# Liz490/multimodal_alzheimer

Hardware: AMD Instinct MI355X
Metric: volumes/sec fwd+bwd, 3D-ResNet-10 @128^3 bf16, 1/2/4/8 MI355X; % HBM roofline (higher is better)
Workload: dtype bf16; 1 GPU; BASELINE config 2: Anat_CNN ResNet-10 MRI-only, 1x128^3, batch 8/GPU, weighted CE, Adam, fwd+bwd+step; global_batch=8, parallelism=dp1, step_launch=hip graph replay

## Files before the change

### multimodal_alzheimer_amd/csrc/conv.hip

```cpp
#include <cstring>

#include "common.h"
#include "reduce.h"
#include "patchconv.h"
#include "pointwise.h"
#include "stem.h"

namespace {

constexpr int MAXTAPS = 344;
constexpr int TAPB = ((3 * MAXTAPS * 4 + 15) / 16) * 16;
constexpr int RB = 128;

struct Geom {
  int M, Nd, Cs, K, Kpad, cs_shift, taps, nb;
  int Ds, Hs, Ws, Dd, Hd, Wd;
  int KD, KH, KW;
  int sd, sh, sw, pd, ph, pw, dd, dh, dw;
  const void* res;
  int relu;
};

enum { FWD = 0, DGRAD = 1 };

// ... 1271 lines not shown
        return launch_igemm_bm<T, 128, MODE, 256, 4, 2, 2>(g, m_max, classes, src, w, bias,
                                                          dst, stats, st);
      if (cfg == 5)
        return launch_igemm_bm<T, 256, MODE, 256, 2, 4, 4, 64>(g, m_max, classes, src, w, bias,
                                                              dst, stats, st);
      if (cfg == 6)
        return launch_igemm_bm<T, 256, MODE, 256, 2, 4, 3, 64>(g, m_max, classes, src, w, bias,
                                                              dst, stats, st);
    }
  }
  const bool small = igemm_bm(m_max * classes, g) == 64;
  if constexpr (sizeof(T) == 2) {
    if (igemm_nst(g, MODE) == 3) {
      if (bn_of(g) == 64)
        return small ? launch_igemm_bm<T, 64, MODE, 64, 2, 2, 3>(g, m_max, classes, src, w, bias, dst, stats, st)
                     : launch_igemm_bm<T, 64, MODE, 128, 2, 2, 3>(g, m_max, classes, src, w, bias, dst, stats, st);
      return small ? launch_igemm_bm<T, 128, MODE, 64, 2, 2, 3>(g, m_max, classes, src, w, bias, dst, stats, st)
                   : launch_igemm_bm<T, 128, MODE, 128, 2, 2, 3>(g, m_max, classes, src, w, bias, dst, stats, st);
    }
  }
  if (bn_of(g) == 64)
    return small ? launch_igemm_bm<T, 64, MODE, 64>(g, m_max, classes, src, w, bias, dst, stats, st)
                 : launch_igemm_bm<T, 64, MODE, 128>(g, m_max, classes, src, w, bias, dst, stats, st);
  return small ? launch_igemm_bm<T, 128, MODE, 64>(g, m_max, classes, src, w, bias, dst, stats, st)
               : launch_igemm_bm<T, 128, MODE, 128>(g, m_max, classes, src, w, bias, dst, stats, st);
}

template <int MODE>
int run_igemm(const Geom& g, int dtype, int64_t m_max, int classes, const void* src,
              const void* w, const float* bias, void* dst, float* stats, hipStream_t st) {
  if (dtype == MMAD_BF16)
    return run_igemm_t<u16, MODE>(g, m_max, classes, src, w, bias, dst, stats, st);
  return run_igemm_t<float, MODE>(g, m_max, classes, src, w, bias, dst, stats, st);
}

int wgrad_xcd() {
  static const int v = [] { const char* e = getenv("MMAD_WGRAD_XCD"); return e ? atoi(e) : 1; }();
  return v;
}

template <typename T, int BMW, int WBK, int NST, int WBNT, int WGM, int WGN, bool XFIX>
int launch_wgrad_x(const Geom& g, const WSplit& sp, const void* x, const void* dy, float* ws,
                   hipStream_t st) {
  const size_t lds = TAPB + NST * WBK * (BMW + WBNT) * sizeof(T);
  static const bool ok = set_lds(wgrad_kernel<T, BMW, WBK, NST, WBNT, WGM, WGN, XFIX>, lds);
  if (!ok) return MMAD_EUNSUPPORTED;
  const uint32_t xb = (uint32_t)((int64_t)g.nb * g.Ds * g.Hs * g.Ws * g.Cs * sizeof(T));
  const uint32_t yb = (uint32_t)((int64_t)g.M * g.Nd * sizeof(T));
  dim3 grid((unsigned)cdiv(g.K, WBNT), (unsigned)cdiv(g.Nd, BMW), (unsigned)sp.splits);
  hipLaunchKernelGGL((wgrad_kernel<T, BMW, WBK, NST, WBNT, WGM, WGN, XFIX>), grid,
                     dim3(64 * WGM * WGN), lds, st, g, (const T*)x, (const T*)dy, ws,
                     sp.m_per_split, xb, yb, wgrad_xcd());
  return launch_status();
}

template <typename T, int BMW, int WBK, int NST, int WBNT = WBN, int WGM = 2, int WGN = 2>
int launch_wgrad_k(const Geom& g, const WSplit& sp, const void* x, const void* dy, float* ws,
                   hipStream_t st) {
  if ((int64_t)g.nb * g.Ds * g.Hs * g.Ws * g.Cs * (int64_t)sizeof(T) >= (int64_t(1) << 31) ||
      (int64_t)g.M * g.Nd * (int64_t)sizeof(T) >= (int64_t(1) << 31))
    return MMAD_EUNSUPPORTED;
  if (WBK % g.Wd == 0)
    return launch_wgrad_x<T, BMW, WBK, NST, WBNT, WGM, WGN, true>(g, sp, x, dy, ws, st);
  return launch_wgrad_x<T, BMW, WBK, NST, WBNT, WGM, WGN, false>(g, sp, x, dy, ws, st);
}

int wgrad_1x1_nst() {
  static const int v = [] { const char* e = getenv("MMAD_WGRAD_1X1_NST"); return e ? atoi(e) : 3; }();
  return v;
}

template <typename T, int BMW>
int launch_wgrad(const Geom& g, const WSplit& sp, const void* x, const void* dy, float* ws,
                 hipStream_t st) {
  if (g.taps == 1 && wgrad_1x1_nst() == 3) return launch_wgrad_k<T, BMW, 32, 3>(g, sp, x, dy, ws, st);
  return launch_wgrad_k<T, BMW, 32, 2>(g, sp, x, dy, ws, st);
}

unsigned grid_for(int64_t total, int block = 256) {
  return (unsigned)std::max<int64_t>(1, std::min<int64_t>(cdiv(total, block), 65536));
}

enum Leaf { STEM, LATTICE5, LATTICE_ZP, LATTICE, LATTICE8, PATCHZ, PATCH, S2, PW, IGEMM, NONE };
enum Epi { EPI_NONE, EPI_RES, EPI_BNSUM };
bool leaf_has(Leaf l, Epi e) {
  if (e == EPI_RES) return l != STEM && l != PW;
  if (e == EPI_BNSUM) return l == LATTICE_ZP || l == LATTICE8 || l == PATCH;
  return true;
}
struct Route { Leaf leaf; int64_t tiles; };

Route resolve(const mmad_conv_desc* d, const Geom& g, int dtype, Epi epi, bool launch = true) {
  const Route none{NONE, -1};
  auto pick = [&](Leaf l, int64_t tiles) { return leaf_has(l, epi) ? Route{l, tiles} : none; };
  const bool u = d != nullptr && unfolded(d);
  if (u && epi != EPI_NONE) return none;
  if (u && mmad_stem::fwd_ok(d, dtype) && stem_kernel_on())
    return pick(STEM, mmad_stem::fwd_stats_rows(d));
  if (launch && !geom_ok(g, dtype)) return none;
  if (!u && dtype == MMAD_BF16) {
    const mmad_patch::Geo q = patch_geo(g);
    if (g.sd == 1 && g.sh == 1 && g.sw == 1) {
      if (mmad_lattice5::ok(q)) return pick(LATTICE5, mmad_lattice5::tiles(q));
      const bool zp = mmad_lattice_zp::ok(q);
      const int64_t lt = zp ? mmad_lattice_zp::tiles(q) : mmad_lattice::tiles(q);
      if (mmad_lattice::ok(q, lt)) return pick(zp ? LATTICE_ZP : LATTICE, lt);
      if (mmad_lattice8::ok(q)) return pick(LATTICE8, mmad_lattice8::tiles(q));
      if (mmad_patch::ok(q))
        return mmad_patchz::ok(q) ? pick(PATCHZ, mmad_patchz::tiles(q))
                                  : pick(PATCH, mmad_patch::tiles(q));
    }
    if (mmad_s2::ok(q, g.sd, g.sh, g.sw)) return pick(S2, mmad_s2::tiles(q));
  }
  if (d != nullptr && leaf_has(PW, epi) && mmad_pw::fwd_ok(d, dtype))
    return pick(PW, mmad_pw::fwd_tiles(d));
  return pick(IGEMM, cdiv(g.M, fwd_tile_rows(g, dtype)));
}

int launch_route(const Route& r, const mmad_conv_desc* d, const Geom& g, int dtype,
                 const mmad_patch::Geo& q, const void* x, const void* wp, const float* bias,
                 void* y, float* stats, void* stream) {
  switch (r.leaf) {
    case STEM: return mmad_stem::fwd(d, x, wp, bias, y, stats, stream);
    case LATTICE5: return mmad_lattice5::fwd(q, x, wp, bias, y, stats, stream);
    case LATTICE_ZP: return mmad_lattice_zp::fwd(q, x, wp, bias, y, stats, stream);
    case LATTICE: return mmad_lattice::fwd(q, x, wp, bias, y, stats, stream);
    case LATTICE8: return mmad_lattice8::fwd(q, x, wp, bias, y, stats, stream);
    case PATCHZ: return mmad_patchz::fwd(q, x, wp, bias, y, stats, stream);
    case PATCH: return mmad_patch::fwd(q, x, wp, bias, y, stats, stream);
    case S2: return mmad_s2::fwd(q, g.sd, g.sh, g.sw, x, wp, bias, y, stats, stream);
    case PW: return mmad_pw::fwd(d, x, wp, bias, y, stats, stream);
    case IGEMM: return run_igemm<FWD>(g, dtype, g.M, 1, x, wp, bias, y, stats, as_stream(stream));
    case NONE: break;
  }
  return MMAD_EUNSUPPORTED;
}

Route dgrad_fwd_route(const mmad_conv_desc* d, int dtype, Epi epi, Geom* gf) {
  if (!desc_ok(d) || (dtype != MMAD_F32 && dtype != MMAD_BF16) || unfolded(d) ||
      mmad_pw::ok(d, dtype) || !dgrad_as_fwd(d))
    return Route{NONE, -1};
  *gf = dgrad_fwd_geom(d, dtype);
  return resolve(nullptr, *gf, dtype, epi);
}

}

extern "C" {

int mmad_set_kernel_variant(const char* name, int value) {
  if (name == nullptr) return -1;
  if (std::strcmp(name, "lattice_zp") == 0) return mmad_lattice_zp::set_mode(value);
  if (std::strcmp(name, "lattice") == 0) return mmad_lattice::set_mode(value);
  if (std::strcmp(name, "lattice8") == 0) return mmad_lattice8::set_mode(value);
  if (std::strcmp(name, "lattice8_xwalk") == 0) return mmad_lattice8::set_xwalk(value);
  if (std::strcmp(name, "lattice5") == 0) return mmad_lattice5::set_mode(value);
  if (std::strcmp(name, "pool_run") == 0) return mmad_pool::set_run_mode(value);
  if (std::strcmp(name, "patchz") == 0) return mmad_patchz::set_mode(value);
  if (std::strcmp(name, "pw_wg3_dedup") == 0) return mmad_pw::set_wg3_dedup(value);
  return -1;
}

int64_t mmad_conv_packed_elems(const mmad_conv_desc* d, int dtype, int for_dgrad) {
  if (!desc_ok(d)) return -1;
  const Geom g = for_dgrad ? dgrad_geom(d, dtype) : fwd_geom(d, dtype);
  return (int64_t)g.Nd * g.Kpad;
}

int mmad_conv_pack_weight_scaled(const mmad_conv_desc* d, int dtype, const float* w,
                                 const float* scale, void* wp, int for_dgrad, void* stream);

int mmad_conv_pack_weight(const mmad_conv_desc* d, int dtype, const float* w, void* wp,
                          int for_dgrad, void* stream) {
  return mmad_conv_pack_weight_scaled(d, dtype, w, nullptr, wp, for_dgrad, stream);
}

int mmad_conv_pack_weight_scaled(const mmad_conv_desc* d, int dtype, const float* w,
                                 const float* scale, void* wp, int for_dgrad, void* stream) {
  if (!desc_ok(d)) return MMAD_EBADSHAPE;
  if (dtype != MMAD_F32 && dtype != MMAD_BF16) return MMAD_EBADDTYPE;
  if (!w || !wp) return MMAD_ENULL;
  if (for_dgrad && unfolded(d)) return MMAD_EUNSUPPORTED;
  const Geom g = for_dgrad ? dgrad_geom(d, dtype) : fwd_geom(d, dtype);
  if (!geom_ok(g, dtype)) return MMAD_EUNSUPPORTED;
  const int mode = for_dgrad ? 1 : (unfolded(d) ? 2 : 0);
  const int flip = for_dgrad && dgrad_as_fwd(d);
  const int64_t total = (int64_t)g.Nd * g.Kpad;
  if (scale != nullptr && (mode != 0 || g.Kpad != g.K)) return MMAD_EUNSUPPORTED;
  if (mode != 2 && g.Kpad == g.K) {
    const int R = mode == 0 ? d->ci : d->co;
    const int Cc = mode == 0 ? g.taps : d->ci * g.taps;
    const int B = mode == 0 ? d->co : 1;
    const int64_t ob = mode == 0 ? g.Kpad : 0, oj1 = mode == 0 ? 0 : g.Kpad;
    const int jd = g.taps, oj2 = mode == 0 ? d->ci : d->co;
    dim3 grid((unsigned)cdiv(Cc, 64), (unsigned)cdiv(R, 64), (unsigned)B);
    if (dtype == MMAD_BF16)
      hipLaunchKernelGGL(pack_transpose_kernel<u16>, grid, dim3(256), 0, as_stream(stream), w,
                         (u16*)wp, R, Cc, ob, jd, oj1, oj2, flip, scale);
    else
      hipLaunchKernelGGL(pack_transpose_kernel<float>, grid, dim3(256), 0, as_stream(stream), w,
                         (float*)wp, R, Cc, ob, jd, oj1, oj2, flip, scale);
    return launch_status();
  }
  if (dtype == MMAD_BF16)
    hipLaunchKernelGGL(pack_weight_kernel<u16>, dim3(grid_for(total)), dim3(256), 0,
                       as_stream(stream), w, (u16*)wp, g.Nd, g.Kpad, g.K, g.Cs, g.cs_shift,
                       g.taps, mode, d->ci, d->kw, flip);
  else
    hipLaunchKernelGGL(pack_weight_kernel<float>, dim3(grid_for(total)), dim3(256), 0,
                       as_stream(stream), w, (float*)wp, g.Nd, g.Kpad, g.K, g.Cs, g.cs_shift,
                       g.taps, mode, d->ci, d->kw, flip);
  return launch_status();
}

int mmad_conv_pack_job(const mmad_conv_desc* d, int dtype, int for_dgrad, const float* w,
                       void* wp, int64_t tile0, mmad_pack_job* job) {
  if (!desc_ok(d)) return MMAD_EBADSHAPE;
  if (dtype != MMAD_F32 && dtype != MMAD_BF16) return MMAD_EBADDTYPE;
  if (!w || !wp || !job) return MMAD_ENULL;
  if (unfolded(d)) return MMAD_EUNSUPPORTED;
  const Geom g = for_dgrad ? dgrad_geom(d, dtype) : fwd_geom(d, dtype);
  if (!geom_ok(g, dtype) || g.Kpad != g.K) return MMAD_EUNSUPPORTED;
  const bool fw = !for_dgrad;
  mmad_pack_job j{};
  j.w = w;
  j.w_packed = wp;
  j.rows = fw ? d->co * d->ci : d->co;
  j.rdiv = fw ? d->ci : d->co;
  j.cols = fw ? g.taps : d->ci * g.taps;
  j.batch = 1;
  j.jdiv = g.taps;
  j.ostride_j2 = fw ? d->ci : d->co;
  j.ostride_b = fw ? g.Kpad : 0;
  j.ostride_j1 = fw ? 0 : g.Kpad;
  const bool narrow = j.cols <= 32;
  j.tiles_x = (int)cdiv(j.cols, narrow ? 32 : 64);
  j.tiles_y = (int)cdiv(j.rows, narrow ? 128 : 64);
  j.pad_ = for_dgrad && dgrad_as_fwd(d);
  j.tile0 = tile0;
  *job = j;
  return MMAD_OK;
}

int mmad_conv_pack_dual_job(const mmad_conv_desc* d, int dtype, const float* w, void* w_fwd,
                            void* w_dgrad, int64_t tile0, mmad_pack_dual* job) {
  if (!desc_ok(d)) return MMAD_EBADSHAPE;
  if (dtype != MMAD_BF16) return MMAD_EUNSUPPORTED;
  if (!w || !w_fwd || !w_dgrad || !job) return MMAD_ENULL;
  if (unfolded(d)) return MMAD_EUNSUPPORTED;
  const Geom gf = fwd_geom(d, dtype), gd = dgrad_geom(d, dtype);
  if (!geom_ok(gf, dtype) || !geom_ok(gd, dtype) || gf.Kpad != gf.K || gd.Kpad != gd.K)
    return MMAD_EUNSUPPORTED;
  if (d->ci % 16 || d->co % 16 || gf.taps > 27) return MMAD_EUNSUPPORTED;
  mmad_pack_dual j{};
  j.w = w;
  j.w_fwd = w_fwd;
  j.w_dgrad = w_dgrad;
  j.co = d->co;
  j.ci = d->ci;
  j.taps = gf.taps;
  j.flip = dgrad_as_fwd(d) ? 1 : 0;
  j.tile0 = tile0;
  *job = j;
  return MMAD_OK;
}

int64_t mmad_pack_dual_tiles(const mmad_pack_dual* job) {
  return job ? (int64_t)(job->co / 16) * (job->ci / 16) : -1;
}

int mmad_conv_pack_dual_batch(int dtype, int njobs, const mmad_pack_dual* jobs,
                              int64_t total_tiles, void* stream) {
  if (njobs <= 0 || total_tiles <= 0 || total_tiles > INT32_MAX) return MMAD_EBADSHAPE;
  if (!jobs) return MMAD_ENULL;
  if (dtype != MMAD_BF16) return MMAD_EBADDTYPE;
  hipLaunchKernelGGL(pack_dual_kernel, dim3((unsigned)total_tiles), dim3(256), 0,
                     as_stream(stream), jobs, njobs);
  return launch_status();
}

int64_t mmad_pack_job_tiles(const mmad_pack_job* job) {
  return job ? (int64_t)job->tiles_x * job->tiles_y * job->batch : -1;
}

int mmad_conv_pack_batch(int dtype, int njobs, const mmad_pack_job* jobs, int64_t total_tiles,
                         void* stream) {
  if (njobs <= 0 || total_tiles <= 0 || total_tiles > INT32_MAX) return MMAD_EBADSHAPE;
  if (!jobs) return MMAD_ENULL;
  if (dtype == MMAD_BF16)
    hipLaunchKernelGGL(pack_batch_kernel<u16>, dim3((unsigned)total_tiles), dim3(256), 0,
                       as_stream(stream), jobs, njobs);
  else if (dtype == MMAD_F32)
    hipLaunchKernelGGL(pack_batch_kernel<float>, dim3((unsigned)total_tiles), dim3(256), 0,
                       as_stream(stream), jobs, njobs);
  else
    return MMAD_EBADDTYPE;
  return launch_status();
}

int64_t mmad_conv_unfolded_elems(const mmad_conv_desc* d) {
  if (!desc_ok(d) || !unfolded(d)) return -1;
  return (int64_t)d->n * d->di * d->hi * d->wo * 8;
}

int mmad_conv_unfold_input(const mmad_conv_desc* d, int in_dtype, const void* x, int dtype,
                           void* xu, void* stream) {
// ... 379 lines not shown
```

### multimodal_alzheimer_amd/csrc/latticeconv.hip

```cpp
#include <algorithm>
#include <atomic>
#include <cstdlib>
#include <type_traits>

#include "common.h"
#include "patchconv.h"

namespace {

constexpr int S = 4;
constexpr int NS = 32;
constexpr int PL = S * S * NS;
constexpr int RBL = 64;
constexpr int KC = RBL / 2;
constexpr int PLANE = PL * RBL;
constexpr int BNL = 128;
constexpr int TPS = 3;
constexpr int BTAP = BNL * RBL;
constexpr int BSLOT = TPS * BTAP;
#ifndef LAT_NSTL
#define LAT_NSTL 3
#endif
constexpr int NSTL = LAT_NSTL;
constexpr int NPS = 2;
// ... 202 lines not shown
  };
  auto run = [&](auto wmc) {
    constexpr int WM = decltype(wmc)::value;
    for (int u = 0; u < ngrp; ++u) {
      const char* apl = smem + (u % NPS) * PLANE + a_lane;
      const int s0 = u * 3;
      const bool py = u >= 1 && u + 1 < ngrp;
      one_stage(s0, std::integral_constant<int, 0>{}, py);
      stage_body<TN, WM, -1>(acc, ring + (s0 % NSTL) * BSLOT + b_lane, apl);
      one_stage(s0 + 1, std::integral_constant<int, 1>{}, py);
      stage_body<TN, WM, 0>(acc, ring + ((s0 + 1) % NSTL) * BSLOT + b_lane, apl);
      one_stage(s0 + 2, std::integral_constant<int, 2>{}, py);
      stage_body<TN, WM, 1>(acc, ring + ((s0 + 2) % NSTL) * BSLOT + b_lane, apl);
    }
  };
  if (g.prio && wave >= 4) __builtin_amdgcn_s_setprio(1);
  switch (wm) {
    case 0: run(std::integral_constant<int, 0>{}); break;
    case 1: run(std::integral_constant<int, 1>{}); break;
    case 2: run(std::integral_constant<int, 2>{}); break;
    default: run(std::integral_constant<int, 3>{}); break;
  }
  __syncthreads();

  auto dst_vox = [&](int row) -> int64_t {
    const int pos = row / NS, s = row % NS;
    const int q = q0 + s;
    const int rz = q / (d * d), ry = (q / d) % d, rx = q % d;
    const int ty = pos / S, tx = pos % S;
    if constexpr (RAG) {
      const int z = rz + d * tz, y = ry + d * ty, x = rx + d * tx;
      if (z >= g.D || y >= g.H || x >= g.W) return -1;
      return (((int64_t)n * g.D + z) * g.H + y) * g.W + x;
    }
    return (((int64_t)n * E + rz + d * tz) * E + ry + d * ty) * E + rx + d * tx;
  };
  u16* ctile = reinterpret_cast<u16*>(smem);
  uint32_t vmask = 0xffffffffu;
  if constexpr (RAG) {
    vmask = 0;
#pragma unroll 1
    for (int b = 0; b < 32; ++b) {
      const int i = b >> 3, h = (b >> 2) & 1, e = b & 3;
      const int row = (i * S + ((i + wm) & 3)) * NS + h * 16 + lk * 4 + e;
      if (dst_vox(row) >= 0) vmask |= 1u << b;
    }
  }
  float cs[TN], cq[TN];
#pragma unroll
  for (int j = 0; j < TN; ++j) {
    cs[j] = 0.f;
    cq[j] = 0.f;
    const int col = wn * 16 * TN + j * 16 + lr;
    const float bv = bias != nullptr ? bias[n0 + col] : 0.f;
#pragma unroll
    for (int i = 0; i < 4; ++i) {
      const int pos = i * S + ((i + wm) & 3);
#pragma unroll
      for (int h = 0; h < 2; ++h)
#pragma unroll
        for (int e = 0; e < 4; ++e) {
          const int row = pos * NS + h * 16 + lk * 4 + e;
          const float v = acc[i * 2 + h][j][e] + bv;
          ctile[row * (CROW / 2) + col] = f2bf(v);
          if ((vmask >> (i * 8 + h * 4 + e)) & 1u) {
            cs[j] += v;
            cq[j] += v * v;
          }
        }
    }
  }
  __syncthreads();
  constexpr int CPR = BW / 8;
#pragma unroll
  for (int hh = 0; hh < PL * CPR / NTHR; ++hh) {
    const int qd = tid + NTHR * hh;
    const int row = qd / CPR, c8 = qd % CPR;
    const int64_t dv = dst_vox(row);
    if (RAG && dv < 0) continue;
    const int64_t o = dv * g.Nd + n0 + c8 * 8;
    u32x4 v = *reinterpret_cast<const u32x4*>(reinterpret_cast<const char*>(ctile) + row * CROW +
                                              c8 * 16);
    if (g.res != nullptr || g.relu) v = epi_res_relu(v, g.res ? g.res + o : nullptr, g.relu);
    *reinterpret_cast<u32x4*>(dst + o) = v;
  }
  if (stats != nullptr) {
    float* red = reinterpret_cast<float*>(smem + PL * CROW);
#pragma unroll
    for (int j = 0; j < TN; ++j) {
      cs[j] += __shfl_xor(cs[j], 16, 64);
      cs[j] += __shfl_xor(cs[j], 32, 64);
      cq[j] += __shfl_xor(cq[j], 16, 64);
      cq[j] += __shfl_xor(cq[j], 32, 64);
    }
    if (wm > 0 && lk == 0) {
#pragma unroll
      for (int j = 0; j < TN; ++j) {
        const int col = wn * 16 * TN + j * 16 + lr;
        red[(wm - 1) * 2 * BW + col] = cs[j];
        red[(wm - 1) * 2 * BW + BW + col] = cq[j];
      }
    }
    __syncthreads();
    if (wm == 0 && lk == 0) {
      const int mt = gid * NZ + tz;
#pragma unroll
      for (int j = 0; j < TN; ++j) {
        const int col = wn * 16 * TN + j * 16 + lr;
        float ss = cs[j], qs = cq[j];
        for (int w = 1; w < 4; ++w) {
          ss += red[(w - 1) * 2 * BW + col];
          qs += red[(w - 1) * 2 * BW + BW + col];
        }
        stats[((int64_t)mt * 2) * g.Nd + n0 + col] = ss;
        stats[((int64_t)mt * 2 + 1) * g.Nd + n0 + col] = qs;
      }
    }
  }
}


constexpr int WXROW = 64;
constexpr int WYROW = 128;
constexpr int WPLANE = PL * WXROW;
constexpr int WXSLOTS = 4;
constexpr int WYST = 2 * NS * WYROW;
constexpr int WYSLOTS = 3;
constexpr int WZERO_OFF = WXSLOTS * WPLANE;
constexpr int WY_OFF = WZERO_OFF + NS * WXROW;
constexpr int WLDS = WY_OFF + WYSLOTS * WYST;

__device__ __forceinline__ int wsz64(int r) { return 2 * ((r >> 3) & 1); }
__device__ __forceinline__ int wsz128(int r) { return 2 * ((r >> 1) & 1) + 4 * ((r >> 3) & 1); }

template <int ROWB>
__device__ __forceinline__ bf16x8 tr_frag(const char* img, int r0, int col) {
  const int ch = col >> 3, hb = (col & 7) * 2;
  const int r1 = r0 + 4;
  const int s0 = ROWB == 64 ? wsz64(r0) : wsz128(r0);
  const int s1 = ROWB == 64 ? wsz64(r1) : wsz128(r1);
  bf16x4 lo = __builtin_amdgcn_ds_read_tr16_b64_v4bf16(
      (LDS_AS bf16x4*)(img + r0 * ROWB + ((ch ^ s0) << 4) + hb));
  bf16x4 hi = __builtin_amdgcn_ds_read_tr16_b64_v4bf16(
      (LDS_AS bf16x4*)(img + r1 * ROWB + ((ch ^ s1) << 4) + hb));
  return __builtin_shufflevector(lo, hi, 0, 1, 2, 3, 4, 5, 6, 7);
}

struct LWG {
  int nb, Cs, Nd, d, K;
  int groups_per_split;
  uint32_t xbytes, ybytes;
};

template <int DD>
__global__ __launch_bounds__(NTHR) void lattice_wgrad_kernel(LWG g, const u16* __restrict__ src,
                                                             const u16* __restrict__ dy,
                                                             float* __restrict__ ws) {
  extern __shared__ __attribute__((aligned(16))) char smem[];
  const int tid = threadIdx.x, lane = tid & 63;
  const int wave = __builtin_amdgcn_readfirstlane(tid >> 6);
  const int nci = g.Cs / KC, nco = g.Nd / 64;
  const int nwg = gridDim.x, bid = blockIdx.x;
  const int xcd = bid & 7, qq = nwg >> 3, rr = nwg & 7;
  const int tile = (xcd < rr ? xcd * (qq + 1) : rr * (qq + 1) + (xcd - rr) * qq) + (bid >> 3);
  const int cot = tile % nco;
  const int t2 = tile / nco;
  const int cit = t2 % nci, split = t2 / nci;
  const int co0 = cot * 64, ci0 = cit * KC;
  constexpr int d = DD, E = S * d;
  const int gpn = d * d * d / NS;
  const int g0 = split * g.groups_per_split;
  const int nplane_out = g.groups_per_split * S;
  const int nstage = nplane_out * 8;
  const int64_t plane_vox = (int64_t)d * E * E;

  auto grp_vox = [&](int gi, int z, int ty, int tx) -> int64_t {
    const int n = gi / gpn, q = (gi % gpn) * NS;
    const int rz = q / (d * d), ry = (q / d) % d, rx = q % d;
    return (((int64_t)n * E + rz + d * z) * E + ry + d * ty) * E + rx + d * tx;
  };
  auto sub_part = [&](int s) -> int64_t {
    const int q = s;
    const int rz = q / (d * d), ry = (q / d) % d, rx = q % d;
    return ((int64_t)rz * E + ry) * E + rx;
  };
  const int xrow_l = lane >> 2;
  const __amdgpu_buffer_rsrc_t rsx = __builtin_amdgcn_make_buffer_rsrc(
      (void*)src, 0, (int)__builtin_amdgcn_readfirstlane(g.xbytes), 0x00020000);
  const __amdgpu_buffer_rsrc_t rsy = __builtin_amdgcn_make_buffer_rsrc(
      (void*)dy, 0, (int)__builtin_amdgcn_readfirstlane(g.ybytes), 0x00020000);
  const uint32_t lds0 = lds_addr_of(smem);
  uint32_t xlane[4];
#pragma unroll
  for (int k = 0; k < 4; ++k) {
    const int row = (wave * 4 + k) * 16 + xrow_l;
    const int pos = row / NS, sb = row % NS;
    const int chunk = (lane & 3) ^ wsz64(row);
    xlane[k] = (uint32_t)(((sub_part(sb) + (int64_t)d * (pos / S) * E + d * (pos % S)) * g.Cs +
                           ci0 + chunk * 8) * 2);
  }
  auto issue_x = [&](int e) {
    const int gi = g0 + e / S, pz = e % S;
    const uint32_t slot = lds0 + (uint32_t)(((unsigned)e % WXSLOTS) * WPLANE);
    const uint32_t zb = (uint32_t)(grp_vox(gi, pz, 0, 0) * g.Cs * 2);
#pragma unroll
    for (int k = 0; k < 4; ++k)
      buf_lds16_asm(zb + xlane[k], rsx, slot + (uint32_t)((wave * 4 + k) * 1024));
  };
  const int yrow = wave * 8 + (lane >> 3);
  const int ychunk = (lane & 7) ^ wsz128(yrow);
  const uint32_t ylane = (uint32_t)(((sub_part(yrow % NS) + (int64_t)d * (yrow / NS)) * g.Nd +
                                     co0 + ychunk * 8) * 2);


  const int cf = wave & 1, tg = wave >> 1;
  const int t0 = tg * 7, nt = tg == 3 ? 6 : 7;
  const int lk = lane >> 4, q4 = (lane & 15) >> 2, p4 = lane & 3;
  const int rsel = 8 * lk + q4;
  f32x4 acc[4][7];
#pragma unroll
  for (int i = 0; i < 4; ++i)
#pragma unroll
    for (int k = 0; k < 7; ++k) acc[i][k] = f32x4{0.f, 0.f, 0.f, 0.f};

  auto tr_off = [&](int rowb, int r, int col, int sw) -> uint32_t {
    return (uint32_t)(r * rowb + ((((col >> 3) ^ sw)) << 4) + (col & 7) * 2);
  };
  uint32_t ya_lo[4], ya_hi[4];
#pragma unroll
  for (int i = 0; i < 4; ++i) {
    const int col = i * 16 + 4 * p4;
    ya_lo[i] = tr_off(WYROW, rsel, col, wsz128(rsel));
    ya_hi[i] = tr_off(WYROW, rsel + 4, col, wsz128(rsel + 4));
  }
  const uint32_t xb_lo = tr_off(WXROW, rsel, cf * 16 + 4 * p4, wsz64(rsel));
  const uint32_t xb_hi = tr_off(WXROW, rsel + 4, cf * 16 + 4 * p4, wsz64(rsel + 4));
  auto tr8 = [](const char* p) {
    return __builtin_amdgcn_ds_read_tr16_b64_v4bf16((LDS_AS bf16x4*)p);
  };
  auto issue_y_at = [&](int64_t plane_vox0, int m, int sl) {
    const uint32_t base =
        (uint32_t)((plane_vox0 + (int64_t)d * (m / 2) * E + 2 * d * (m % 2)) * g.Nd * 2);
    buf_lds16_asm(base + ylane, rsy, lds0 + (uint32_t)(WY_OFF + sl * WYST + wave * 1024));
  };
  auto plane_y0 = [&](int o) -> int64_t { return grp_vox(g0 + o / S, o % S, 0, 0); };

  issue_x(0);
  issue_x(1);
  issue_y_at(plane_y0(0), 0, 0);
  issue_y_at(plane_y0(0), 1, 1);

  struct WFr { bf16x8 a[4], b[7]; };
  auto run = [&](auto tgc) {
    constexpr int TG = decltype(tgc)::value;
    constexpr int NT = TG == 3 ? 6 : 7;
    auto yx_on = [](auto kc, auto posc) constexpr {
      constexpr int K = decltype(kc)::value, POS = decltype(posc)::value;
      constexpr int t = TG * 7 + K;
      constexpr int ky = (t / 3) % 3 - 1, kx = t % 3 - 1;
      constexpr int py = POS / S + ky, px = POS % S + kx;
      return K < NT && py >= 0 && py < S && px >= 0 && px < S;
    };
    auto z_on = [](auto kc, auto tzc) constexpr {
      constexpr int K = decltype(kc)::value, TZ = decltype(tzc)::value;
      constexpr int kz = (TG * 7 + K) / 9 - 1;
      return TZ + kz >= 0 && TZ + kz < S;
    };
    auto kread = [&](const char* yimg, auto qc, auto posc, auto tzc, WFr& f) {
      constexpr int Q = decltype(qc)::value, POS = decltype(posc)::value;
      constexpr int TZ = decltype(tzc)::value;
#pragma unroll
      for (int i = 0; i < 4; ++i)
        f.a[i] = __builtin_shufflevector(tr8(yimg + Q * NS * WYROW + ya_lo[i]),
                                         tr8(yimg + Q * NS * WYROW + ya_hi[i]), 0, 1, 2, 3, 4,
                                         5, 6, 7);
      auto one = [&](auto kc) {
        constexpr int K = decltype(kc)::value;
        if constexpr (yx_on(kc, posc) && z_on(kc, tzc)) {
          constexpr int t = TG * 7 + K;
          constexpr int dk = (t / 9 - 1) * WPLANE + (((t / 3) % 3 - 1) * S + t % 3 - 1) * NS * WXROW +
                             POS * NS * WXROW;
          const char* img = smem + TZ * WPLANE + dk;
          f.b[K] = __builtin_shufflevector(tr8(img + xb_lo), tr8(img + xb_hi), 0, 1, 2, 3, 4, 5,
                                           6, 7);
        }
      };
      one(std::integral_constant<int, 0>{});
      one(std::integral_constant<int, 1>{});
      one(std::integral_constant<int, 2>{});
      one(std::integral_constant<int, 3>{});
      one(std::integral_constant<int, 4>{});
      one(std::integral_constant<int, 5>{});
      one(std::integral_constant<int, 6>{});
    };
    auto kmma = [&](const WFr& f, auto posc, auto tzc) {
      auto one = [&](auto kc) {
        constexpr int K = decltype(kc)::value;
        if constexpr (yx_on(kc, posc) && z_on(kc, tzc)) {
#pragma unroll
          for (int i = 0; i < 4; ++i)
            acc[i][K] = __builtin_amdgcn_mfma_f32_16x16x32_bf16(f.a[i], f.b[K], acc[i][K], 0, 0,
                                                                0);
        }
      };
      one(std::integral_constant<int, 0>{});
      one(std::integral_constant<int, 1>{});
      one(std::integral_constant<int, 2>{});
      one(std::integral_constant<int, 3>{});
      one(std::integral_constant<int, 4>{});
      one(std::integral_constant<int, 5>{});
      one(std::integral_constant<int, 6>{});
    };

    auto plane = [&](int o, auto tzc) {
      const bool xnow = o + 2 < nplane_out;
      const int64_t y_here = plane_y0(o);
      const int64_t y_next = o + 1 < nplane_out ? plane_y0(o + 1) : y_here;
      const int sl0 = (int)((unsigned)(o * 8) % WYSLOTS);
      auto stage = [&](auto mc) {
        constexpr int M = decltype(mc)::value;
        const int sl = (int)((unsigned)(sl0 + M) % WYSLOTS);
        const bool last = o + 1 == nplane_out && M == 7;
        if ((M == 1 || M == 2) && xnow) wait_vm_lgkm0<5>();
        else if (last) wait_vm_lgkm0<0>();
        else wait_vm_lgkm0<1>();
        raw_barrier();
        if (M < 6) issue_y_at(y_here, M + 2, (int)((unsigned)(sl + 2) % WYSLOTS));
        else if (o + 1 < nplane_out) issue_y_at(y_next, M - 6, (int)((unsigned)(sl + 2) % WYSLOTS));
        if (M == 0 && xnow) issue_x(o + 2);
        int yoff = WY_OFF + sl * WYST;
        asm volatile("" : "+s"(yoff));
        const char* yimg = smem + yoff;
        WFr f0, f1;
        kread(yimg, std::integral_constant<int, 0>{}, std::integral_constant<int, 2 * M>{}, tzc,
              f0);
        kread(yimg, std::integral_constant<int, 1>{}, std::integral_constant<int, 2 * M + 1>{},
              tzc, f1);
        kmma(f0, std::integral_constant<int, 2 * M>{}, tzc);
        kmma(f1, std::integral_constant<int, 2 * M + 1>{}, tzc);
      };
      stage(std::integral_constant<int, 0>{});
      stage(std::integral_constant<int, 1>{});
      stage(std::integral_constant<int, 2>{});
      stage(std::integral_constant<int, 3>{});
      stage(std::integral_constant<int, 4>{});
      stage(std::integral_constant<int, 5>{});
      stage(std::integral_constant<int, 6>{});
      stage(std::integral_constant<int, 7>{});
    };
    for (int og = 0; og < nplane_out; og += S) {
      plane(og + 0, std::integral_constant<int, 0>{});
      plane(og + 1, std::integral_constant<int, 1>{});
      plane(og + 2, std::integral_constant<int, 2>{});
      plane(og + 3, std::integral_constant<int, 3>{});
    }
  };
  switch (tg) {
    case 0: run(std::integral_constant<int, 0>{}); break;
    case 1: run(std::integral_constant<int, 1>{}); break;
    case 2: run(std::integral_constant<int, 2>{}); break;
    default: run(std::integral_constant<int, 3>{}); break;
  }

  float* out = ws + (int64_t)split * g.Nd * g.K;
  const int lr = lane & 15;
#pragma unroll
  for (int k = 0; k < 7; ++k) {
    if (k < nt) {
      const int kcol = (t0 + k) * g.Cs + ci0 + cf * 16 + lr;
#pragma unroll
      for (int i = 0; i < 4; ++i)
#pragma unroll
        for (int r = 0; r < 4; ++r)
          out[(int64_t)(co0 + i * 16 + lk * 4 + r) * g.K + kcol] = acc[i][k][r];
    }
  }
}

std::atomic<int> g_lattice_mode{-1};
int lattice_mode() {
  int v = g_lattice_mode.load(std::memory_order_relaxed);
  if (v < 0) {
    const char* e = getenv("MMAD_LATTICE");
    int expect = -1;
    g_lattice_mode.compare_exchange_strong(expect, e ? atoi(e) : 1);
    v = g_lattice_mode.load(std::memory_order_relaxed);
  }
  return v;
}

}

namespace mmad_lattice {

int set_mode(int v) {
  const int prev = lattice_mode();
  if (v >= 0) g_lattice_mode.store(v, std::memory_order_relaxed);
  return prev;
}

static bool exact(const mmad_patch::Geo& q) {
  const int E = S * q.dd;
  return q.Ds == E && q.Hs == E && q.Ws == E && q.Dd == E && q.Hd == E && q.Wd == E;
}
static int ragged_mode() {
  static const int v = [] {
    const char* e = getenv("MMAD_LATTICE_RAGGED");
    return e ? atoi(e) : 1;
  }();
  return v;
}
static bool ragged(const mmad_patch::Geo& q) {
  const int d = q.dd;
  return !exact(q) && q.Ds == q.Dd && q.Hs == q.Hd && q.Ws == q.Wd &&
         (q.Hs + d - 1) / d <= S && (q.Ws + d - 1) / d <= S &&
         (int64_t)q.Ds * q.Hs * q.Ws * q.Cs * 2 < (int64_t(1) << 31);
}
static int planes(const mmad_patch::Geo& q) {
  return exact(q) ? S : (q.Ds + q.dd - 1) / q.dd;
}

bool ok(const mmad_patch::Geo& q, int64_t fill_tiles) {
  if (lattice_mode() <= 0) return false;
  const int d = q.dd;
  if (q.KD != 3 || q.KH != 3 || q.KW != 3 || q.dh != d || q.dw != d || d < 2) return false;
  if (q.pd != d || q.ph != d || q.pw != d) return false;
  const int E = S * d;
  if (!exact(q) && !(ragged_mode() > 0 && ragged(q))) return false;
  if ((d * d * d) % NS) return false;
  if (q.Cs % KC || q.Nd % 64 || q.Kpad != 27 * q.Cs) return false;
  if ((int64_t)E * E * E * q.Cs >= (int64_t(1) << 31) ||
      (int64_t)q.Nd * q.Kpad >= (int64_t(1) << 31))
    return false;
  if (lattice_mode() == 1 && fill_tiles * (q.Nd / 64) < 256) return false;
  return (int64_t)q.nb * E * E * E * q.Cs < (int64_t(1) << 40);
}

int64_t tiles(const mmad_patch::Geo& q) {
  return (int64_t)q.nb * q.dd * q.dd * q.dd / NS * planes(q);
}

int wgrad_splits(const mmad_patch::Geo& q) {
  const int64_t tiles = (int64_t)(q.Cs / KC) * (q.Nd / 64);
  const int ngroups = q.nb * q.dd * q.dd * q.dd / NS;
  int sp = 1;
  while (tiles * sp < 256 && ngroups % (sp * 2) == 0) sp *= 2;
  return sp;
}

int lattice_wgrad_mode() {
  static const int v = [] {
    const char* e = getenv("MMAD_LATTICE_WGRAD");
    return e ? atoi(e) : 1;
  }();
  return v;
}

bool wgrad_ok(const mmad_patch::Geo& q) {
  if (lattice_mode() <= 0 || lattice_wgrad_mode() <= 0) return false;
  const int d = q.dd;
  if (q.KD != 3 || q.KH != 3 || q.KW != 3 || q.dh != d || q.dw != d || d < 2) return false;
  if (q.pd != d || q.ph != d || q.pw != d) return false;
  const int E = S * d;
  if (q.Ds != E || q.Hs != E || q.Ws != E || q.Dd != E || q.Hd != E || q.Wd != E) return false;
  if ((d * d * d) % NS || q.Cs % KC || q.Nd % 64 || (d != 4 && d != 8)) return false;
  const int64_t tiles = (int64_t)(q.Cs / KC) * (q.Nd / 64) * wgrad_splits(q);
  if (lattice_mode() == 1 && tiles < 256) return false;
  return (int64_t)q.nb * E * E * E * std::max(q.Cs, q.Nd) * 2 < (int64_t(1) << 31);
}

int64_t wgrad_workspace(const mmad_patch::Geo& q) {
  return (int64_t)wgrad_splits(q) * q.Nd * 27 * q.Cs * 4;
}

int wgrad(const mmad_patch::Geo& q, const void* x, const void* dy, float* ws, int* splits,
          void* stream) {
  if (!wgrad_ok(q)) return MMAD_EUNSUPPORTED;
  static const bool attr =
      hipFuncSetAttribute((const void*)lattice_wgrad_kernel<4>,
                          hipFuncAttributeMaxDynamicSharedMemorySize, WLDS) == hipSuccess &&
      hipFuncSetAttribute((const void*)lattice_wgrad_kernel<8>,
                          hipFuncAttributeMaxDynamicSharedMemorySize, WLDS) == hipSuccess;
  if (!attr) return MMAD_EUNSUPPORTED;
  const int sp = wgrad_splits(q);
  LWG g{};
  g.nb = q.nb; g.Cs = q.Cs; g.Nd = q.Nd; g.d = q.dd; g.K = 27 * q.Cs;
  g.groups_per_split = q.nb * q.dd * q.dd * q.dd / NS / sp;
  const int64_t vox = (int64_t)q.nb * S * q.dd * S * q.dd * S * q.dd;
  g.xbytes = (uint32_t)(vox * q.Cs * 2);
  g.ybytes = (uint32_t)(vox * q.Nd * 2);
  const int64_t nblk = (int64_t)(q.Cs / KC) * (q.Nd / 64) * sp;
  if (q.dd == 4)
    hipLaunchKernelGGL(lattice_wgrad_kernel<4>, dim3((unsigned)nblk), dim3(NTHR), WLDS,
                       as_stream(stream), g, (const u16*)x, (const u16*)dy, ws);
  else
    hipLaunchKernelGGL(lattice_wgrad_kernel<8>, dim3((unsigned)nblk), dim3(NTHR), WLDS,
                       as_stream(stream), g, (const u16*)x, (const u16*)dy, ws);
  *splits = sp;
  return launch_status();
}

int fwd(const mmad_patch::Geo& q, const void* src, const void* wp, const float* bias,
        void* dst, float* stats, void* stream) {
  if (!mmad_lattice::ok(q, mmad_lattice::tiles(q))) return MMAD_EUNSUPPORTED;
  if (q.bny != nullptr) return MMAD_EUNSUPPORTED;
  const bool rag = !exact(q);
  static const bool attr =
      hipFuncSetAttribute((const void*)lattice_conv_kernel<4, false>,
                          hipFuncAttributeMaxDynamicSharedMemorySize, LDS_BYTES) == hipSuccess &&
      hipFuncSetAttribute((const void*)lattice_conv_kernel<2, false>,
                          hipFuncAttributeMaxDynamicSharedMemorySize, LDS_BYTES) == hipSuccess &&
      hipFuncSetAttribute((const void*)lattice_conv_kernel<4, true>,
                          hipFuncAttributeMaxDynamicSharedMemorySize, LDS_BYTES) == hipSuccess &&
      hipFuncSetAttribute((const void*)lattice_conv_kernel<2, true>,
                          hipFuncAttributeMaxDynamicSharedMemorySize, LDS_BYTES) == hipSuccess;
  if (!attr) return MMAD_EUNSUPPORTED;
  const bool wide = q.Nd % BNL == 0 && mmad_lattice::tiles(q) * (q.Nd / BNL) >= 256;
  LG g{};
  g.nb = q.nb; g.Cs = q.Cs; g.Nd = q.Nd; g.Kpad = q.Kpad; g.d = q.dd;
  g.ngroups = q.nb * q.dd * q.dd * q.dd / NS;
  g.nbn = q.Nd / (wide ? BNL : 64);
  g.nchunk = q.Cs / KC;
  g.res = reinterpret_cast<const u16*>(q.res);
  g.relu = q.relu;
  static const int prio = [] {
    const char* e = getenv("MMAD_SETPRIO");
    return e ? atoi(e) : 0;
  }();
  g.prio = prio;
  g.D = q.Ds; g.H = q.Hs; g.W = q.Ws;
  g.nz = planes(q);
  const int64_t nblk = (int64_t)g.ngroups * g.nz * g.nbn;
  auto go = [&](auto kern) {
    hipLaunchKernelGGL(kern, dim3((unsigned)nblk), dim3(NTHR), LDS_BYTES, as_stream(stream), g,
                       (const u16*)src, (const u16*)wp, bias, (u16*)dst, stats);
  };
  if (wide) rag ? go(lattice_conv_kernel<4, true>) : go(lattice_conv_kernel<4, false>);
  else rag ? go(lattice_conv_kernel<2, true>) : go(lattice_conv_kernel<2, false>);
  return launch_status();
}

}
```

### multimodal_alzheimer_amd/csrc/patchconv.h

```cpp
#pragma once
#include <stdint.h>

#include "../../include/mmad.h"

namespace mmad_patch {
struct Geo {
  int nb, Cs, Nd, Kpad;
  int Ds, Hs, Ws, Dd, Hd, Wd;
  int KD, KH, KW, pd, ph, pw, dd, dh, dw;
  const void* res = nullptr;
  int relu = 0;
  const void* bny = nullptr;
  const float* bnsc = nullptr;
  const float* bnsh = nullptr;
  const float* bnmu = nullptr;
  const float* bnis = nullptr;
  float* bnparts = nullptr;
};
bool ok(const Geo& g);
int64_t tiles(const Geo& g);
int fwd(const Geo& g, const void* src, const void* wp, const float* bias, void* dst,
        float* stats, void* stream);
}

namespace mmad_patchz {
int set_mode(int v);
bool ok(const mmad_patch::Geo& g);
int64_t tiles(const mmad_patch::Geo& g);
int fwd(const mmad_patch::Geo& g, const void* src, const void* wp, const float* bias, void* dst,
        float* stats, void* stream);
}

namespace mmad_lattice {
int set_mode(int v);
bool ok(const mmad_patch::Geo& g, int64_t fill_tiles);
int64_t tiles(const mmad_patch::Geo& g);
int fwd(const mmad_patch::Geo& g, const void* src, const void* wp, const float* bias, void* dst,
        float* stats, void* stream);
bool wgrad_ok(const mmad_patch::Geo& g);
int64_t wgrad_workspace(const mmad_patch::Geo& g);
int wgrad(const mmad_patch::Geo& g, const void* x, const void* dy, float* ws, int* splits,
          void* stream);
}

namespace mmad_s2 {
bool ok(const mmad_patch::Geo& g, int sd, int sh, int sw);
int64_t tiles(const mmad_patch::Geo& g);
int fwd(const mmad_patch::Geo& g, int sd, int sh, int sw, const void* src, const void* wp,
        const float* bias, void* dst, float* stats, void* stream);
bool dgrad_ok(const mmad_conv_desc* d);
int dgrad(const mmad_conv_desc* d, const void* dy, const void* wpt, void* dx, void* stream);
}

namespace mmad_lattice_zp {
int set_mode(int v);
bool ok(const mmad_patch::Geo& g);
int64_t tiles(const mmad_patch::Geo& g);
int fwd(const mmad_patch::Geo& g, const void* src, const void* wp, const float* bias, void* dst,
        float* stats, void* stream);
}

namespace mmad_lattice5 {
int set_mode(int v);
bool ok(const mmad_patch::Geo& g);
int64_t tiles(const mmad_patch::Geo& g);
int fwd(const mmad_patch::Geo& g, const void* src, const void* wp, const float* bias, void* dst,
        float* stats, void* stream);
bool wgrad_ok(const mmad_patch::Geo& g);
int64_t wgrad_workspace(const mmad_patch::Geo& g);
int wgrad(const mmad_patch::Geo& g, const void* x, const void* dy, float* ws, int* splits,
          void* stream);
}

namespace mmad_lattice8 {
int set_mode(int v);
int set_xwalk(int v);
bool ok(const mmad_patch::Geo& g);
int64_t tiles(const mmad_patch::Geo& g);
int fwd(const mmad_patch::Geo& g, const void* src, const void* wp, const float* bias, void* dst,
        float* stats, void* stream);
}

namespace mmad_pwgrad {
bool ok(const mmad_patch::Geo& g);
int64_t workspace(const mmad_patch::Geo& g);
int wgrad(const mmad_patch::Geo& g, const void* x, const void* dy, float* ws, int* splits,
          void* stream);
}

namespace mmad_pool {
int set_run_mode(int v);
}
```

Measured before the change: 2823 volumes/sec.

## Add rebalanced, software-pipelined lattice wgrad kernel form with compile-time tap pruning

```diff
diff --git a/multimodal_alzheimer_amd/csrc/conv.hip b/multimodal_alzheimer_amd/csrc/conv.hip
--- a/multimodal_alzheimer_amd/csrc/conv.hip
+++ b/multimodal_alzheimer_amd/csrc/conv.hip
@@ -1447,6 +1447,7 @@
   if (name == nullptr) return -1;
   if (std::strcmp(name, "lattice_zp") == 0) return mmad_lattice_zp::set_mode(value);
   if (std::strcmp(name, "lattice") == 0) return mmad_lattice::set_mode(value);
+  if (std::strcmp(name, "lattice_wgrad_form") == 0) return mmad_lattice::set_wgrad_form(value);
   if (std::strcmp(name, "lattice8") == 0) return mmad_lattice8::set_mode(value);
   if (std::strcmp(name, "lattice8_xwalk") == 0) return mmad_lattice8::set_xwalk(value);
   if (std::strcmp(name, "lattice5") == 0) return mmad_lattice5::set_mode(value);
diff --git a/multimodal_alzheimer_amd/csrc/latticeconv.hip b/multimodal_alzheimer_amd/csrc/latticeconv.hip
--- a/multimodal_alzheimer_amd/csrc/latticeconv.hip
+++ b/multimodal_alzheimer_amd/csrc/latticeconv.hip
@@ -378,7 +378,51 @@
   uint32_t xbytes, ybytes;
 };
 
-template <int DD>
+#ifdef LWG_DEAL_OLD
+constexpr int LWG_DEAL[4][7] = {{0, 1, 2, 3, 4, 5, 6},
+                                {7, 8, 9, 10, 11, 12, 13},
+                                {14, 15, 16, 17, 18, 19, 20},
+                                {21, 22, 23, 24, 25, 26, -1}};
+#else
+constexpr int LWG_DEAL[4][7] = {{0, 5, 6, 10, 17, 22, 24},
+                                {4, 8, 9, 11, 15, 21, 23},
+                                {1, 7, 12, 14, 18, 20, 25},
+                                {2, 3, 13, 16, 19, 26, -1}};
+#endif
+constexpr bool lwg_live(int tg, int k, int pos, int tz) {
+  const int t = LWG_DEAL[tg][k];
+  if (t < 0) return false;
+  const int pz = tz + t / 9 - 1, py = pos / S + (t / 3) % 3 - 1, px = pos % S + t % 3 - 1;
+  return pz >= 0 && pz < S && py >= 0 && py < S && px >= 0 && px < S;
+}
+constexpr int lwg_nlive(int tg, int pos, int tz) {
+  int n = 0;
+  for (int k = 0; k < 7; ++k) n += lwg_live(tg, k, pos, tz);
+  return n;
+}
+constexpr bool lwg_deal_ok() {
+  int seen[27] = {};
+  for (int g = 0; g < 4; ++g)
+    for (int k = 0; k < 7; ++k) {
+      const int t = LWG_DEAL[g][k];
+      if (t < 0 ? (g != 3 || k != 6) : (t >= 27 || seen[t]++)) return false;
+    }
+  return true;
+}
+static_assert(lwg_deal_ok(), "LWG_DEAL is not a deal of the 27 taps into 7 / 7 / 7 / 6");
+
+template <int NM, int NR>
+__device__ __forceinline__ void lwg_interleave() {
+#pragma unroll
+  for (int k = 0; k < (NM < NR ? NM : NR); ++k) {
+    __builtin_amdgcn_sched_group_barrier(0x008, 1, 0);
+    __builtin_amdgcn_sched_group_barrier(0x100, 1, 0);
+  }
+  if constexpr (NM > NR) __builtin_amdgcn_sched_group_barrier(0x008, NM - NR, 0);
+  if constexpr (NR > NM) __builtin_amdgcn_sched_group_barrier(0x100, NR - NM, 0);
+}
+
+template <int DD, int FORM>
 __global__ __launch_bounds__(NTHR) void lattice_wgrad_kernel(LWG g, const u16* __restrict__ src,
                                                              const u16* __restrict__ dy,
                                                              float* __restrict__ ws) {
@@ -425,13 +469,25 @@
     xlane[k] = (uint32_t)(((sub_part(sb) + (int64_t)d * (pos / S) * E + d * (pos % S)) * g.Cs +
                            ci0 + chunk * 8) * 2);
   }
-  auto issue_x = [&](int e) {
+  const uint32_t xlane0 = (uint32_t)((sub_part(xrow_l) * g.Cs + ci0 +
+                                      ((lane & 3) ^ wsz64(xrow_l)) * 8) * 2);
+  constexpr uint32_t LWG_OOB = 0x80000000u;
+  auto issue_x = [&](int e, bool real = true) {
     const int gi = g0 + e / S, pz = e % S;
     const uint32_t slot = lds0 + (uint32_t)(((unsigned)e % WXSLOTS) * WPLANE);
-    const uint32_t zb = (uint32_t)(grp_vox(gi, pz, 0, 0) * g.Cs * 2);
-#pragma unroll
-    for (int k = 0; k < 4; ++k)
-      buf_lds16_asm(zb + xlane[k], rsx, slot + (uint32_t)((wave * 4 + k) * 1024));
+    const uint32_t zb = real ? (uint32_t)(grp_vox(gi, pz, 0, 0) * g.Cs * 2) : LWG_OOB;
+#pragma unroll
+    for (int k = 0; k < 4; ++k) {
+      if constexpr (FORM == 0) {
+        buf_lds16_asm(zb + xlane[k], rsx, slot + (uint32_t)((wave * 4 + k) * 1024));
+      } else {
+        const int pos = (wave * 4 + k) >> 1;
+        uint32_t sk = zb + (uint32_t)(((sub_part(16 * (k & 1)) + (int64_t)d * (pos / S) * E +
+                                        d * (pos % S)) * g.Cs) * 2);
+        asm volatile("" : "+s"(sk));
+        buf_lds16_asm(sk + xlane0, rsx, slot + (uint32_t)((wave * 4 + k) * 1024));
+      }
+    }
   };
   const int yrow = wave * 8 + (lane >> 3);
   const int ychunk = (lane & 7) ^ wsz128(yrow);
@@ -464,9 +520,10 @@
   auto tr8 = [](const char* p) {
     return __builtin_amdgcn_ds_read_tr16_b64_v4bf16((LDS_AS bf16x4*)p);
   };
-  auto issue_y_at = [&](int64_t plane_vox0, int m, int sl) {
+  auto issue_y_at = [&](int64_t plane_vox0, int m, int sl, bool real = true) {
     const uint32_t base =
-        (uint32_t)((plane_vox0 + (int64_t)d * (m / 2) * E + 2 * d * (m % 2)) * g.Nd * 2);
+        real ? (uint32_t)((plane_vox0 + (int64_t)d * (m / 2) * E + 2 * d * (m % 2)) * g.Nd * 2)
+             : LWG_OOB;
     buf_lds16_asm(base + ylane, rsy, lds0 + (uint32_t)(WY_OFF + sl * WYST + wave * 1024));
   };
   auto plane_y0 = [&](int o) -> int64_t { return grp_vox(g0 + o / S, o % S, 0, 0); };
@@ -581,6 +638,143 @@
       plane(og + 3, std::integral_constant<int, 3>{});
     }
   };
+  auto run1 = [&](auto tgc) {
+    constexpr int TG = decltype(tgc)::value;
+    auto each_tap = [](auto&& fn) {
+      [&]<int... K>(std::integer_sequence<int, K...>) {
+        (fn(std::integral_constant<int, K>{}), ...);
+      }(std::make_integer_sequence<int, 7>{});
+    };
+    auto read_a = [&](const char* yimg, auto qc, bf16x8 (&a)[4]) {
+      constexpr int Q = decltype(qc)::value;
+#pragma unroll
+      for (int i = 0; i < 4; ++i)
+        a[i] = __builtin_shufflevector(tr8(yimg + Q * NS * WYROW + ya_lo[i]),
+                                       tr8(yimg + (Q * NS + 4) * WYROW + ya_lo[i]), 0, 1, 2, 3,
+                                       4, 5, 6, 7);
+    };
+    auto read_b = [&](auto posc, auto tzc, bf16x8 (&b)[7], uint32_t xb_hi64) {
+      constexpr int POS = decltype(posc)::value, TZ = decltype(tzc)::value;
+      each_tap([&](auto kc) {
+        constexpr int K = decltype(kc)::value;
+        if constexpr (lwg_live(TG, K, POS, TZ)) {
+          constexpr int t = LWG_DEAL[TG][K];
+          constexpr int dk = (t / 9 - 1) * WPLANE + (((t / 3) % 3 - 1) * S + t % 3 - 1) * NS * WXROW +
+                             POS * NS * WXROW;
+          constexpr int off = TZ * WPLANE + dk;
+          const char* img = off < 0x10000 ? smem + off + xb_lo : smem + (off - 0x10000) + xb_hi64;
+          b[K] = __builtin_shufflevector(tr8(img), tr8(img + 4 * WXROW), 0, 1, 2, 3, 4, 5, 6, 7);
+        }
+      });
+    };
+    auto x_hi64 = [&]() {
+      int o = 0x10000;
+      asm volatile("" : "+s"(o));
+      return xb_lo + (uint32_t)o;
+    };
+    auto kmma = [&](const bf16x8 (&a)[4], const bf16x8 (&b)[7], auto posc, auto tzc) {
+      constexpr int POS = decltype(posc)::value, TZ = decltype(tzc)::value;
+      each_tap([&](auto kc) {
+        constexpr int K = decltype(kc)::value;
+        if constexpr (lwg_live(TG, K, POS, TZ)) {
+#pragma unroll
+          for (int i = 0; i < 4; ++i)
+            acc[i][K] = __builtin_amdgcn_mfma_f32_16x16x32_bf16(a[i], b[K], acc[i][K], 0, 0, 0);
+        }
+      });
+    };
+    bf16x8 b0[7];
+#ifndef LWG_NO_ROLL
+    wait_vm_lgkm0<1>();
+    raw_barrier();
+    read_b(std::integral_constant<int, 0>{}, std::integral_constant<int, 0>{}, b0, x_hi64());
+#endif
+
+    auto plane = [&](int o, auto tzc) {
+      constexpr int TZ = decltype(tzc)::value;
+      const bool xnow = o + 2 < nplane_out;
+      const int64_t y_here = plane_y0(o);
+      const int64_t y_next = o + 1 < nplane_out ? plane_y0(o + 1) : y_here;
+      const int sl0 = (int)((unsigned)(o * 8) % WYSLOTS);
+      auto stage = [&](auto mc) {
+        constexpr int M = decltype(mc)::value;
+        const int sl = (int)((unsigned)(sl0 + M) % WYSLOTS);
+        if constexpr (M == 1 || M == 2) wait_vm_lgkm0<5>();
+        else wait_vm_lgkm0<1>();
+        raw_barrier();
+        issue_y_at(M < 6 ? y_here : y_next, (M + 2) & 7, (int)((unsigned)(sl + 2) % WYSLOTS),
+                   M < 6 || o + 1 < nplane_out);
+        if constexpr (M == 0) issue_x(o + 2, xnow);
+        int yoff = WY_OFF + sl * WYST;
+        asm volatile("" : "+s"(yoff));
+        const char* yimg = smem + yoff;
+        constexpr std::integral_constant<int, 0> q0{};
+        constexpr std::integral_constant<int, 1> q1{};
+        constexpr std::integral_constant<int, 2 * M> p0{};
+        constexpr std::integral_constant<int, 2 * M + 1> p1{};
+        bf16x8 a0[4], a1[4], b1[7];
+        const uint32_t xh = x_hi64();
+#ifdef LWG_NO_ROLL
+        read_a(yimg, q0, a0);
+        read_b(p0, tzc, b0, xh);
+        read_a(yimg, q1, a1);
+        read_b(p1, tzc, b1, xh);
+        kmma(a0, b0, p0, tzc);
+        kmma(a1, b1, p1, tzc);
+#else
+        constexpr std::integral_constant<int, (M < 7 ? 2 * M + 2 : 0)> np{};
+        constexpr std::integral_constant<int, (M < 7 ? TZ : (TZ + 1) % S)> ntz{};
+        constexpr int N0 = lwg_nlive(TG, 2 * M, TZ), N1 = lwg_nlive(TG, 2 * M + 1, TZ);
+        constexpr int NN = lwg_nlive(TG, decltype(np)::value, decltype(ntz)::value);
+        __builtin_amdgcn_sched_barrier(0);
+        read_a(yimg, q0, a0);
+        read_a(yimg, q1, a1);
+        read_b(p1, tzc, b1, xh);
+        kmma(a0, b0, p0, tzc);
+        __builtin_amdgcn_sched_group_barrier(0x100, 8, 0);
+        lwg_interleave<4 * N0, 8 + 2 * N1>();
+        __builtin_amdgcn_sched_barrier(0);
+        read_b(np, ntz, b0, xh);
+        kmma(a1, b1, p1, tzc);
+        lwg_interleave<4 * N1, 2 * NN>();
+        __builtin_amdgcn_sched_barrier(0);
+#endif
+      };
+      [&]<int... M>(std::integer_sequence<int, M...>) {
+        (stage(std::integral_constant<int, M>{}), ...);
+      }(std::make_integer_sequence<int, 8>{});
+    };
+    for (int og = 0; og < nplane_out; og += S) {
+      plane(og + 0, std::integral_constant<int, 0>{});
+      plane(og + 1, std::integral_constant<int, 1>{});
+      plane(og + 2, std::integral_constant<int, 2>{});
+      plane(og + 3, std::integral_constant<int, 3>{});
+    }
+    wait_vm_lgkm0<0>();
+    float* out = ws + (int64_t)split * g.Nd * g.K;
+    const int el = (int)__builtin_amdgcn_mbcnt_hi(~0u, __builtin_amdgcn_mbcnt_lo(~0u, 0u));
+    const int lr = el & 15, lk = el >> 4;
+    each_tap([&](auto kc) {
+      constexpr int K = decltype(kc)::value;
+      if constexpr (LWG_DEAL[TG][K] >= 0) {
+        const int kcol = LWG_DEAL[TG][K] * g.Cs + ci0 + cf * 16 + lr;
+#pragma unroll
+        for (int i = 0; i < 4; ++i)
+#pragma unroll
+          for (int r = 0; r < 4; ++r)
+            out[(int64_t)(co0 + i * 16 + lk * 4 + r) * g.K + kcol] = acc[i][K][r];
+      }
+    });
+  };
+  if constexpr (FORM == 1) {
+    switch (tg) {
+      case 0: run1(std::integral_constant<int, 0>{}); break;
+      case 1: run1(std::integral_constant<int, 1>{}); break;
+      case 2: run1(std::integral_constant<int, 2>{}); break;
+      default: run1(std::integral_constant<int, 3>{}); break;
+    }
+    return;
+  }
   switch (tg) {
     case 0: run(std::integral_constant<int, 0>{}); break;
     case 1: run(std::integral_constant<int, 1>{}); break;
@@ -682,6 +876,24 @@
   return v;
 }
 
+std::atomic<int> g_lwg_form{-1};
+int lattice_wgrad_form() {
+  int v = g_lwg_form.load(std::memory_order_relaxed);
+  if (v < 0) {
+    const char* e = getenv("MMAD_LWG_FORM");
+    int expect = -1;
+    g_lwg_form.compare_exchange_strong(expect, e ? (atoi(e) != 0) : 1);
+    v = g_lwg_form.load(std::memory_order_relaxed);
+  }
+  return v;
+}
+
+int set_wgrad_form(int v) {
+  const int prev = lattice_wgrad_form();
+  if (v >= 0) g_lwg_form.store(v != 0, std::memory_order_relaxed);
+  return prev;
+}
+
 bool wgrad_ok(const mmad_patch::Geo& q) {
   if (lattice_mode() <= 0 || lattice_wgrad_mode() <= 0) return false;
   const int d = q.dd;
@@ -703,9 +915,13 @@
           void* stream) {
   if (!wgrad_ok(q)) return MMAD_EUNSUPPORTED;
   static const bool attr =
-      hipFuncSetAttribute((const void*)lattice_wgrad_kernel<4>,
+      hipFuncSetAttribute((const void*)lattice_wgrad_kernel<4, 0>,
                           hipFuncAttributeMaxDynamicSharedMemorySize, WLDS) == hipSuccess &&
-      hipFuncSetAttribute((const void*)lattice_wgrad_kernel<8>,
+      hipFuncSetAttribute((const void*)lattice_wgrad_kernel<8, 0>,
+                          hipFuncAttributeMaxDynamicSharedMemorySize, WLDS) == hipSuccess &&
+      hipFuncSetAttribute((const void*)lattice_wgrad_kernel<4, 1>,
+                          hipFuncAttributeMaxDynamicSharedMemorySize, WLDS) == hipSuccess &&
+      hipFuncSetAttribute((const void*)lattice_wgrad_kernel<8, 1>,
                           hipFuncAttributeMaxDynamicSharedMemorySize, WLDS) == hipSuccess;
   if (!attr) return MMAD_EUNSUPPORTED;
   const int sp = wgrad_splits(q);
@@ -716,12 +932,17 @@
   g.xbytes = (uint32_t)(vox * q.Cs * 2);
   g.ybytes = (uint32_t)(vox * q.Nd * 2);
   const int64_t nblk = (int64_t)(q.Cs / KC) * (q.Nd / 64) * sp;
-  if (q.dd == 4)
-    hipLaunchKernelGGL(lattice_wgrad_kernel<4>, dim3((unsigned)nblk), dim3(NTHR), WLDS,
-                       as_stream(stream), g, (const u16*)x, (const u16*)dy, ws);
-  else
-    hipLaunchKernelGGL(lattice_wgrad_kernel<8>, dim3((unsigned)nblk), dim3(NTHR), WLDS,
-                       as_stream(stream), g, (const u16*)x, (const u16*)dy, ws);
+  auto launch = [&](auto kern) {
+    hipLaunchKernelGGL(kern, dim3((unsigned)nblk), dim3(NTHR), WLDS, as_stream(stream), g,
+                       (const u16*)x, (const u16*)dy, ws);
+  };
+  if (lattice_wgrad_form()) {
+    if (q.dd == 4) launch(lattice_wgrad_kernel<4, 1>);
+    else launch(lattice_wgrad_kernel<8, 1>);
+  } else {
+    if (q.dd == 4) launch(lattice_wgrad_kernel<4, 0>);
+    else launch(lattice_wgrad_kernel<8, 0>);
+  }
   *splits = sp;
   return launch_status();
 }
diff --git a/multimodal_alzheimer_amd/csrc/patchconv.h b/multimodal_alzheimer_amd/csrc/patchconv.h
--- a/multimodal_alzheimer_amd/csrc/patchconv.h
+++ b/multimodal_alzheimer_amd/csrc/patchconv.h
@@ -33,6 +33,7 @@
 
 namespace mmad_lattice {
 int set_mode(int v);
+int set_wgrad_form(int v);
 bool ok(const mmad_patch::Geo& g, int64_t fill_tiles);
 int64_t tiles(const mmad_patch::Geo& g);
 int fwd(const mmad_patch::Geo& g, const void* src, const void* wp, const float* bias, void* dst,
```

Result: no change. 2839 volumes/sec, median of 6 (+0.6%).
